# shamanDevel/IsosurfaceSuperresolution

Hardware: AMD Instinct MI355X
Metric: frames/sec (render+4×SR) at 256³→1080p, 1/2/4/8 GPU; PSNR vs ref (higher is better)
Workload: dtype f32 (fp32 tensors and accumulation; each product as three fp16 MFMAs on split operands, error vs fp64 = the fp32 kernels')

## Files before the change

### isosurfacesuperresolution_amd/csrc/sr_conv_ups3.h

```cpp
#pragma once
#include "sr_split_common.h"

#ifndef U3_LFETCH_ROW
#define U3_LFETCH_ROW 2
#endif
#ifndef U3_SPLANE
#define U3_SPLANE 0
#endif
#ifndef U3_WDMA
#define U3_WDMA 1
#endif
#ifndef U3_CARRY
#define U3_CARRY 2
#endif
#ifndef U3_APREF
#define U3_APREF 0
#endif
#ifndef U3_LR_CS
#define U3_LR_CS 114
#endif

namespace {

constexpr int U3_PART = 2 * SP_PIX;
constexpr int U3_PUNITS = 2 * U3_PART;
constexpr int U3_WROW = 3 * 128;
constexpr int U3_WUNITS = (U3_SPLANE ? 3 : 2) * U3_WROW;
constexpr int U3_LDS_BYTES = (U3_PUNITS + (U3_WDMA ? 2 : 1) * U3_WUNITS) * 16;

__global__ __launch_bounds__(S_THREADS, 3) void conv3x3_split_ups3_kernel(const SplitConvParams p)
{
    extern __shared__ u32x4 patch[];
    u32x4* const wbuf = patch + U3_PUNITS;
    const int tid = threadIdx.x, lane = tid & 63, wave = tid >> 6;
    const int j = lane & 31, h = lane >> 5;
    int bid;
    {
        const int nwg = gridDim.x, q = nwg >> 3, r = nwg & 7, xcd = blockIdx.x & 7;
        bid = (xcd < r ? xcd * (q + 1) : r * (q + 1) + (xcd - r) * q) + (blockIdx.x >> 3);
    }
    const int tx = bid % p.tilesX; bid /= p.tilesX;
    const int ty = bid % p.tilesY, n = bid / p.tilesY;
    const int oy0 = ty * ST_H, ox0 = tx * ST_W;
    const rsrc_t xrs = __builtin_amdgcn_make_buffer_rsrc(const_cast<float*>(p.x + (size_t)n * p.xImage), 0,
                                                         (int)((size_t)p.Cin * p.xPlane * 4), 0x00020000);
    const unsigned planeBytes = (unsigned)p.xPlane * 4u;
    unsigned long long st0 = 0, st1 = 0, st2 = 0;
    if (p.stamps) st0 = __builtin_amdgcn_s_memrealtime();

    const rsrc_t wrs = __builtin_amdgcn_make_buffer_rsrc(const_cast<u32x4*>(p.wq + 1), 0, 9 * p.ksteps * 4096, 0x00020000);
    u32x4* const wdst = wbuf + (tid >> 7) * U3_WROW + (tid & 127);
    u32x4 wreg[3];
    const rsrc_t w3rs = __builtin_amdgcn_make_buffer_rsrc(const_cast<u32x4*>(p.wq + 1 + 9 * p.ksteps * 256), 0, 9 * p.ksteps * 2048, 0x00020000);
    u32x4 wreg3[2];
    auto wfetch = [&](int step) {
        if (step >= 3 * p.ksteps) return;
        const int ks = step / 3, dy = step - 3 * ks;
#pragma unroll
        for (int i = 0; i < 3; ++i) wreg[i] = __builtin_amdgcn_raw_buffer_load_b128(wrs, tid * 16, ((3 * dy + i) * p.ksteps + ks) * 4096, 0);
        if (U3_SPLANE) {
#pragma unroll
            for (int k = 0; k < 2; ++k) {
                const int e = tid + 256 * k;
                wreg3[k] = __builtin_amdgcn_raw_buffer_load_b128(w3rs, (int)(e < 384 ? (unsigned)(e & 127) * 16u : BAD_OFFSET), ((3 * dy + (e >> 7)) * p.ksteps + ks) * 2048, 0);
            }
        }
    };
    auto wpark = [&]() {
#pragma unroll
        for (int i = 0; i < 3; ++i) wdst[i * 128] = wreg[i];
        if (U3_SPLANE) {
            wbuf[2 * U3_WROW + tid] = wreg3[0];
            if (tid < 128) wbuf[2 * U3_WROW + 256 + tid] = wreg3[1];
        }
    };

    constexpr int LR_H = ST_H / 2 + 2, LR_W = ST_W / 2 + 2;
    constexpr int LQ = (ST_W / 2 + 8) / 4;
    constexpr int LUNITS = 16 * LR_H * LQ;
    constexpr int LR_CS = U3_LR_CS;
    constexpr int QR = SP_H / 2, QC = SP_W / 2, UQ = QR * QC;
    float* tmp = reinterpret_cast<float*>(wbuf);
    const int wv = __builtin_amdgcn_readfirstlane(wave);
    auto wdma = [&](int step) {
        if (step >= 3 * p.ksteps) return;
        const int ks = step / 3, dy = step - 3 * ks;
#pragma unroll
        for (int k = 0; k < 3; ++k) {
            const int idx = wv + 4 * k, i = idx >> 2, part = (idx >> 1) & 1, half = idx & 1;
            __builtin_amdgcn_raw_ptr_buffer_load_lds(wrs, (isr_lvoid_t*)(wbuf + (step & 1) * U3_WUNITS + part * U3_WROW + i * 128 + half * 64), 16,
                                                     lane * 16, (((3 * dy + i) * p.ksteps + ks) * 256 + part * 128 + half * 64) * 16, 0, 0);
        }
    };
    const int ly0 = oy0 / 2 - 1, lx0 = ox0 / 2 - 1;
    u32x4 v[3];
    auto lfetch = [&](int cin0) {
#pragma unroll
        for (int k = 0; k < 3; ++k) {
            const int u = tid + k * S_THREADS;
            const int c = u / (LR_H * LQ), rem = u - c * (LR_H * LQ);
            const int r = rem / LQ, q = rem - r * LQ;
            const int iy = ly0 + r, ix = ox0 / 2 - 4 + 4 * q;
            const bool ok = u < LUNITS && (unsigned)iy < (unsigned)p.Hin && (unsigned)ix < (unsigned)p.Win;
            v[k] = __builtin_amdgcn_raw_buffer_load_b128(xrs, (int)(ok ? (unsigned)(cin0 + c) * planeBytes + (unsigned)(iy * p.Win + ix) * 4u
                                                                       : BAD_OFFSET), 0, 0);
        }
    };
    auto lpark = [&]() {
#pragma unroll
        for (int k = 0; k < 3; ++k) {
            const int u = tid + k * S_THREADS;
            if (u >= LUNITS) continue;
            const int c = u / (LR_H * LQ), rem = u - c * (LR_H * LQ);
            const int r = rem / LQ, q = rem - r * LQ;
            const float4 f = __builtin_bit_cast(float4, v[k]);
            float* dst = tmp + c * LR_CS + r * LR_W + 4 * q - 3;
            if (q > 0) dst[0] = f.x;
            if (q > 0 && q < LQ - 1) { dst[1] = f.y; dst[2] = f.z; }
            if (q < LQ - 1) dst[3] = f.w;
        }
    };
    const bool interior = oy0 >= 2 && oy0 + ST_H + 2 <= p.H && ox0 >= 2 && ox0 + ST_W + 2 <= p.W;
    auto interpolate = [&]() {
        _Float16* const patch16 = reinterpret_cast<_Float16*>(patch);
        for (int u = tid; u < 4 * UQ; u += S_THREADS) {
            const int g4 = u & 3, q = u >> 2;
            const int kr = q / QC, kc = q - kr * QC;
            f16x4 h00, h01, h10, h11, l00, l01, l10, l11;
            if (interior) {
                const float* ta = tmp + (g4 * 4) * LR_CS + kr * LR_W + kc;
#pragma unroll
                for (int e = 0; e < 4; ++e) {
                    const float a0 = ta[e * LR_CS], a1 = ta[e * LR_CS + 1];
                    const float b0 = ta[e * LR_CS + LR_W], b1 = ta[e * LR_CS + LR_W + 1];
                    const float al = isr_blend(0.75f, a0, 0.25f, a1), ar = isr_blend(0.25f, a0, 0.75f, a1);
                    const float bl = isr_blend(0.75f, b0, 0.25f, b1), br = isr_blend(0.25f, b0, 0.75f, b1);
                    _Float16 vh, vl;
                    split16x(isr_blend(0.75f, al, 0.25f, bl), vh, vl); h00[e] = vh; l00[e] = vl;
                    split16x(isr_blend(0.75f, ar, 0.25f, br), vh, vl); h01[e] = vh; l01[e] = vl;
                    split16x(isr_blend(0.25f, al, 0.75f, bl), vh, vl); h10[e] = vh; l10[e] = vl;
                    split16x(isr_blend(0.25f, ar, 0.75f, br), vh, vl); h11[e] = vh; l11[e] = vl;
                }
            } else {
                const int Yu = oy0 - 1 + 2 * kr, Xl = ox0 - 1 + 2 * kc;
                const bool oku = (unsigned)Yu < (unsigned)p.H, okd = (unsigned)(Yu + 1) < (unsigned)p.H;
                const bool okl = (unsigned)Xl < (unsigned)p.W, okr = (unsigned)(Xl + 1) < (unsigned)p.W;
                int y0, y1, x0, x1, t0, t1; float lyu, lyd, lxl, lxr, t;
                isr_src_index(oku ? Yu : Yu + 1, 0.5f, p.Hin, y0, y1, t);
                isr_src_index(okl ? Xl : Xl + 1, 0.5f, p.Win, x0, x1, t);
                isr_src_index(Yu, 0.5f, p.Hin, t0, t1, lyu);
                isr_src_index(Yu + 1, 0.5f, p.Hin, t0, t1, lyd);
                isr_src_index(Xl, 0.5f, p.Win, t0, t1, lxl);
                isr_src_index(Xl + 1, 0.5f, p.Win, t0, t1, lxr);
                const float hyu = 1.f - lyu, hyd = 1.f - lyd, hxl = 1.f - lxl, hxr = 1.f - lxr;
                y0 = min(max(y0 - ly0, 0), LR_H - 1); y1 = min(max(y1 - ly0, 0), LR_H - 1);
                x0 = min(max(x0 - lx0, 0), LR_W - 1); x1 = min(max(x1 - lx0, 0), LR_W - 1);
                const float* ta = tmp + (g4 * 4) * LR_CS + y0 * LR_W;
                const float* tb = tmp + (g4 * 4) * LR_CS + y1 * LR_W;
#pragma unroll
                for (int e = 0; e < 4; ++e) {
                    const float a0 = ta[e * LR_CS + x0], a1 = ta[e * LR_CS + x1];
                    const float b0 = tb[e * LR_CS + x0], b1 = tb[e * LR_CS + x1];
                    const float al = isr_blend(hxl, a0, lxl, a1), ar = isr_blend(hxr, a0, lxr, a1);
                    const float bl = isr_blend(hxl, b0, lxl, b1), br = isr_blend(hxr, b0, lxr, b1);
                    _Float16 vh, vl;
                    split16x(isr_blend(hyu, al, lyu, bl), vh, vl); h00[e] = vh; l00[e] = vl;
                    split16x(isr_blend(hyu, ar, lyu, br), vh, vl); h01[e] = vh; l01[e] = vl;
                    split16x(isr_blend(hyd, al, lyd, bl), vh, vl); h10[e] = vh; l10[e] = vl;
                    split16x(isr_blend(hyd, ar, lyd, br), vh, vl); h11[e] = vh; l11[e] = vl;
                }
                const f16x4 z = {(_Float16)0.0f, (_Float16)0.0f, (_Float16)0.0f, (_Float16)0.0f};
                if (!(oku && okl)) { h00 = z; l00 = z; }
                if (!(oku && okr)) { h01 = z; l01 = z; }
                if (!(okd && okl)) { h10 = z; l10 = z; }
                if (!(okd && okr)) { h11 = z; l11 = z; }
            }
            _Float16* d = patch16 + ((size_t)((g4 >> 1) * SP_PIX + (2 * kr) * SP_W + 2 * kc)) * 8 + (g4 & 1) * 4;
            *reinterpret_cast<f16x4*>(d) = h00;
            *reinterpret_cast<f16x4*>(d + 8) = h01;
            *reinterpret_cast<f16x4*>(d + SP_W * 8) = h10;
            *reinterpret_cast<f16x4*>(d + SP_W * 8 + 8) = h11;
            *reinterpret_cast<f16x4*>(d + U3_PART * 8) = l00;
            *reinterpret_cast<f16x4*>(d + U3_PART * 8 + 8) = l01;
            *reinterpret_cast<f16x4*>(d + (U3_PART + SP_W) * 8) = l10;
            *reinterpret_cast<f16x4*>(d + (U3_PART + SP_W) * 8 + 8) = l11;
        }
    };

    f32x16 acc[2][2];
#pragma unroll
    for (int cb = 0; cb < 2; ++cb)
#pragma unroll
        for (int r = 0; r < 2; ++r)
#pragma unroll
            for (int i = 0; i < 16; ++i) acc[cb][r][i] = 0.0f;

    lfetch(0);
    if (U3_WDMA) {
        wdma(0);
#pragma unroll 1
        for (int ks = 0; ks < p.ksteps; ++ks) {
            tmp = reinterpret_cast<float*>(wbuf + ((3 * ks + 1) & 1) * U3_WUNITS);
            lpark();
            __syncthreads();
            if (!(p.dbg & 2)) interpolate();
            f16x8 carry[3], carryo[3];
#pragma unroll
            for (int dy = 0; dy < 3; ++dy) {
                asm volatile("s_waitcnt vmcnt(0)" ::: "memory");
                __syncthreads();
                wdma(3 * ks + dy + 1);
                if (dy == U3_LFETCH_ROW && ks + 1 < p.ksteps) lfetch(16 * (ks + 1));
                if (!(p.dbg & 1)) {
                    const u32x4* wl = wbuf + ((3 * ks + dy) & 1) * U3_WUNITS + h * 64 + j;
                    const u32x4* bl = patch + h * SP_PIX + (wave * 2 + dy) * SP_W + j;
                    f16x8 na0h, na0l, na1h, na1l;
                    if (U3_APREF) {
                        na0h = __builtin_bit_cast(f16x8, wl[0]); na0l = __builtin_bit_cast(f16x8, wl[U3_WROW]);
                        na1h = __builtin_bit_cast(f16x8, wl[32]); na1l = __builtin_bit_cast(f16x8, wl[U3_WROW + 32]);
                    }
#pragma unroll
                    for (int dx = 0; dx < 3; ++dx) {
                        f16x8 a0h, a0l, a1h, a1l;
                        if (U3_APREF) {
                            a0h = na0h; a0l = na0l; a1h = na1h; a1l = na1l;
                            if (dx < 2) {
                                na0h = __builtin_bit_cast(f16x8, wl[(dx + 1) * 128]); na0l = __builtin_bit_cast(f16x8, wl[U3_WROW + (dx + 1) * 128]);
                                na1h = __builtin_bit_cast(f16x8, wl[(dx + 1) * 128 + 32]); na1l = __builtin_bit_cast(f16x8, wl[U3_WROW + (dx + 1) * 128 + 32]);
                                __builtin_amdgcn_sched_barrier(0);
                            }
                        } else {
                            a0h = __builtin_bit_cast(f16x8, wl[dx * 128]);
                            a0l = __builtin_bit_cast(f16x8, wl[U3_WROW + dx * 128]);
                            a1h = __builtin_bit_cast(f16x8, wl[dx * 128 + 32]);
                            a1l = __builtin_bit_cast(f16x8, wl[U3_WROW + dx * 128 + 32]);
                        }
                        const f16x8 a0s = a0h * (_Float16)0.00048828125f;
                        const f16x8 a1s = a1h * (_Float16)0.00048828125f;
#pragma unroll
                        for (int r = 0; r < 2; ++r) {
                            const f16x8 bh = (U3_CARRY && r == 0 && dy > 0) ? carry[dx] : __builtin_bit_cast(f16x8, bl[r * SP_W + dx]);
                            const f16x8 bo = (U3_CARRY == 2 && r == 0 && dy > 0) ? carryo[dx] : __builtin_bit_cast(f16x8, bl[U3_PART + r * SP_W + dx]);
                            if (U3_CARRY && r == 1) carry[dx] = bh;
                            if (U3_CARRY == 2 && r == 1) carryo[dx] = bo;
                            acc[0][r] = mfma16(a0l, bh, acc[0][r]);
                            acc[0][r] = mfma16(a0s, bo, acc[0][r]);
                            acc[0][r] = mfma16(a0h, bh, acc[0][r]);
                            acc[1][r] = mfma16(a1l, bh, acc[1][r]);
                            acc[1][r] = mfma16(a1s, bo, acc[1][r]);
                            acc[1][r] = mfma16(a1h, bh, acc[1][r]);
                        }
                    }
                }
            }
            __syncthreads();
        }
    } else {
    wfetch(0);
#pragma unroll 1
    for (int ks = 0; ks < p.ksteps; ++ks) {
        lpark();
        __syncthreads();
        if (!(p.dbg & 2)) interpolate();
        __syncthreads();
        if (p.stamps && ks == 0) st1 = __builtin_amdgcn_s_memrealtime();
#pragma unroll 1
        for (int dy = 0; dy < 3; ++dy) {
            wpark();
            __syncthreads();
            wfetch(3 * ks + dy + 1);
            if (dy == U3_LFETCH_ROW && ks + 1 < p.ksteps) lfetch(16 * (ks + 1));
            if (!(p.dbg & 1)) {
                const u32x4* wl = wbuf + h * 64 + j;
                const u32x4* bl = patch + h * SP_PIX + (wave * 2 + dy) * SP_W + j;
#pragma unroll
                for (int dx = 0; dx < 3; ++dx) {
                    const f16x8 a0h = __builtin_bit_cast(f16x8, wl[dx * 128]);
                    const f16x8 a0l = __builtin_bit_cast(f16x8, wl[U3_WROW + dx * 128]);
                    const f16x8 a1h = __builtin_bit_cast(f16x8, wl[dx * 128 + 32]);
                    const f16x8 a1l = __builtin_bit_cast(f16x8, wl[U3_WROW + dx * 128 + 32]);
                    const f16x8 a0s = U3_SPLANE ? __builtin_bit_cast(f16x8, wl[2 * U3_WROW + dx * 128]) : a0h * (_Float16)0.00048828125f;
                    const f16x8 a1s = U3_SPLANE ? __builtin_bit_cast(f16x8, wl[2 * U3_WROW + dx * 128 + 32]) : a1h * (_Float16)0.00048828125f;
#pragma unroll
                    for (int r = 0; r < 2; ++r) {
                        const f16x8 bh = __builtin_bit_cast(f16x8, bl[r * SP_W + dx]);
                        const f16x8 bo = __builtin_bit_cast(f16x8, bl[U3_PART + r * SP_W + dx]);
                        acc[0][r] = mfma16(a0l, bh, acc[0][r]);
                        acc[0][r] = mfma16(a0s, bo, acc[0][r]);
                        acc[0][r] = mfma16(a0h, bh, acc[0][r]);
                        acc[1][r] = mfma16(a1l, bh, acc[1][r]);
                        acc[1][r] = mfma16(a1s, bo, acc[1][r]);
                        acc[1][r] = mfma16(a1h, bh, acc[1][r]);
                    }
                }
            }
            __syncthreads();
        }
    }
    }

    if (p.stamps) st2 = __builtin_amdgcn_s_memrealtime();
    if (p.dbg & 8) {
        if (acc[0][0][0] == 123.456f) p.ps[0] = u32x4{1u, 2u, 3u, 4u};
    } else if (p.ps) split_epilogue_ps(p, acc, oy0, ox0, 0, true, wave, j, h);
    else split_epilogue<true>(p, acc, patch, n, oy0, ox0, 0, true, lane, wave, j, h);
    if (p.stamps && tid == 0) {
        asm volatile("s_waitcnt vmcnt(0)" ::: "memory");
        const unsigned long long st3 = __builtin_amdgcn_s_memrealtime();
        unsigned long long* o = p.stamps + (size_t)blockIdx.x * 4;
        o[0] = st0; o[1] = st1; o[2] = st2; o[3] = st3;
    }
}

}

static int isr_launch_split_ups3(const SplitConvParams& p, unsigned nwg, hipStream_t s, hipEvent_t e0, hipEvent_t e1)
{
    if (p.Cin <= 0 || (p.Cin & 15) || p.coutPad != 64 || p.Cout != 64 || p.cgroups != 1 || p.xps) return -1;
    if (!p.ps && ((p.W | p.yPlane | p.rPlane) & 3)) return -1;
    static bool attr = false;
    if (!attr) { (void)hipFuncSetAttribute((const void*)conv3x3_split_ups3_kernel, hipFuncAttributeMaxDynamicSharedMemorySize, U3_LDS_BYTES); attr = true; }
    if (e0 || e1) hipExtLaunchKernelGGL(conv3x3_split_ups3_kernel, dim3(nwg), dim3(S_THREADS), U3_LDS_BYTES, s, e0, e1, 0, p);
    else hipLaunchKernelGGL(conv3x3_split_ups3_kernel, dim3(nwg), dim3(S_THREADS), U3_LDS_BYTES, s, p);
    return hipGetLastError() == hipSuccess ? 0 : -2;
}
```

Before: 600.1.

## Stream low-res input tile into LDS via buffer-load-to-LDS DMA

Adds a U3_LDMA path, on by default, that loads the low-resolution input tile directly into a dedicated LDS staging region with buffer_load_lds. This replaces the register fetch followed by an LDS park, and it drops the end-of-iteration barrier in favour of a waitcnt plus barrier at the top of each k-step. The aim is to free VGPRs and remove the park stores, at the cost of extra LDS per workgroup. A host-side occupancy check refuses to launch if fewer than three blocks fit per CU. The loads are scalar 4-byte per-lane DMAs, which may issue many more memory instructions than the previous 16-byte loads.

```diff
diff --git a/isosurfacesuperresolution_amd/csrc/sr_conv_ups3.h b/isosurfacesuperresolution_amd/csrc/sr_conv_ups3.h
--- a/isosurfacesuperresolution_amd/csrc/sr_conv_ups3.h
+++ b/isosurfacesuperresolution_amd/csrc/sr_conv_ups3.h
@@ -9,6 +9,9 @@
 #endif
 #ifndef U3_WDMA
 #define U3_WDMA 1
+#endif
+#ifndef U3_LDMA
+#define U3_LDMA 1
 #endif
 #ifndef U3_CARRY
 #define U3_CARRY 2
@@ -26,7 +29,10 @@
 constexpr int U3_PUNITS = 2 * U3_PART;
 constexpr int U3_WROW = 3 * 128;
 constexpr int U3_WUNITS = (U3_SPLANE ? 3 : 2) * U3_WROW;
-constexpr int U3_LDS_BYTES = (U3_PUNITS + (U3_WDMA ? 2 : 1) * U3_WUNITS) * 16;
+constexpr int U3_TMP_BYTES = 16 * U3_LR_CS * 4;
+constexpr int U3_LDS_BYTES = (U3_PUNITS + (U3_WDMA ? 2 : 1) * U3_WUNITS) * 16 + (U3_LDMA ? U3_TMP_BYTES : 0);
+static_assert(!U3_LDMA || U3_WDMA, "U3_LDMA is a variant of the U3_WDMA loop");
+static_assert(3 * ((U3_LDS_BYTES + 1279) / 1280 * 1280) <= 163840, "conv3x3_split_ups3_kernel no longer fits a CU three times");
 
 __global__ __launch_bounds__(S_THREADS, 3) void conv3x3_split_ups3_kernel(const SplitConvParams p)
 {
@@ -80,7 +86,7 @@
     constexpr int LUNITS = 16 * LR_H * LQ;
     constexpr int LR_CS = U3_LR_CS;
     constexpr int QR = SP_H / 2, QC = SP_W / 2, UQ = QR * QC;
-    float* tmp = reinterpret_cast<float*>(wbuf);
+    float* tmp = reinterpret_cast<float*>(wbuf + (U3_LDMA ? 2 * U3_WUNITS : 0));
     const int wv = __builtin_amdgcn_readfirstlane(wave);
     auto wdma = [&](int step) {
         if (step >= 3 * p.ksteps) return;
@@ -93,6 +99,23 @@
         }
     };
     const int ly0 = oy0 / 2 - 1, lx0 = ox0 / 2 - 1;
+    unsigned lvoff[2];
+#pragma unroll
+    for (int k = 0; k < 2; ++k) {
+        const int e = lane + 64 * k, r = e / LR_W, iy = ly0 + r, ix = lx0 + e - r * LR_W;
+        const bool ok = e < LR_H * LR_W && (unsigned)iy < (unsigned)p.Hin && (unsigned)ix < (unsigned)p.Win;
+        lvoff[k] = ok ? (unsigned)(iy * p.Win + ix) * 4u : BAD_OFFSET;
+    }
+    auto ldma = [&](int cin0) {
+#pragma unroll
+        for (int c = 0; c < 4; ++c)
+            __builtin_amdgcn_raw_ptr_buffer_load_lds(xrs, (isr_lvoid_t*)(tmp + (4 * wv + c) * LR_CS), 4, (int)lvoff[0], (int)((unsigned)(cin0 + 4 * wv + c) * planeBytes), 0, 0);
+        if (lane < LR_H * LR_W - 64) {
+#pragma unroll
+            for (int c = 0; c < 4; ++c)
+                __builtin_amdgcn_raw_ptr_buffer_load_lds(xrs, (isr_lvoid_t*)(tmp + (4 * wv + c) * LR_CS + 64), 4, (int)lvoff[1], (int)((unsigned)(cin0 + 4 * wv + c) * planeBytes), 0, 0);
+        }
+    };
     u32x4 v[3];
     auto lfetch = [&](int cin0) {
 #pragma unroll
@@ -195,14 +218,19 @@
 #pragma unroll
             for (int i = 0; i < 16; ++i) acc[cb][r][i] = 0.0f;
 
-    lfetch(0);
+    if (U3_LDMA) ldma(0); else lfetch(0);
     if (U3_WDMA) {
         wdma(0);
 #pragma unroll 1
         for (int ks = 0; ks < p.ksteps; ++ks) {
-            tmp = reinterpret_cast<float*>(wbuf + ((3 * ks + 1) & 1) * U3_WUNITS);
-            lpark();
-            __syncthreads();
+            if (U3_LDMA) {
+                asm volatile("s_waitcnt vmcnt(0)" ::: "memory");
+                __syncthreads();
+            } else {
+                tmp = reinterpret_cast<float*>(wbuf + ((3 * ks + 1) & 1) * U3_WUNITS);
+                lpark();
+                __syncthreads();
+            }
             if (!(p.dbg & 2)) interpolate();
             f16x8 carry[3], carryo[3];
 #pragma unroll
@@ -210,7 +238,7 @@
                 asm volatile("s_waitcnt vmcnt(0)" ::: "memory");
                 __syncthreads();
                 wdma(3 * ks + dy + 1);
-                if (dy == U3_LFETCH_ROW && ks + 1 < p.ksteps) lfetch(16 * (ks + 1));
+                if (dy == U3_LFETCH_ROW && ks + 1 < p.ksteps) { if (U3_LDMA) ldma(16 * (ks + 1)); else lfetch(16 * (ks + 1)); }
                 if (!(p.dbg & 1)) {
                     const u32x4* wl = wbuf + ((3 * ks + dy) & 1) * U3_WUNITS + h * 64 + j;
                     const u32x4* bl = patch + h * SP_PIX + (wave * 2 + dy) * SP_W + j;
@@ -253,8 +281,9 @@
                     }
                 }
             }
-            __syncthreads();
-        }
+            if (!U3_LDMA) __syncthreads();
+        }
+        if (U3_LDMA) __syncthreads();
     } else {
     wfetch(0);
 #pragma unroll 1
@@ -319,7 +348,12 @@
     if (p.Cin <= 0 || (p.Cin & 15) || p.coutPad != 64 || p.Cout != 64 || p.cgroups != 1 || p.xps) return -1;
     if (!p.ps && ((p.W | p.yPlane | p.rPlane) & 3)) return -1;
     static bool attr = false;
-    if (!attr) { (void)hipFuncSetAttribute((const void*)conv3x3_split_ups3_kernel, hipFuncAttributeMaxDynamicSharedMemorySize, U3_LDS_BYTES); attr = true; }
+    if (!attr) {
+        (void)hipFuncSetAttribute((const void*)conv3x3_split_ups3_kernel, hipFuncAttributeMaxDynamicSharedMemorySize, U3_LDS_BYTES);
+        int perCU = 0;
+        if (hipOccupancyMaxActiveBlocksPerMultiprocessor(&perCU, (const void*)conv3x3_split_ups3_kernel, S_THREADS, U3_LDS_BYTES) != hipSuccess || perCU < 3) return -2;
+        attr = true;
+    }
     if (e0 || e1) hipExtLaunchKernelGGL(conv3x3_split_ups3_kernel, dim3(nwg), dim3(S_THREADS), U3_LDS_BYTES, s, e0, e1, 0, p);
     else hipLaunchKernelGGL(conv3x3_split_ups3_kernel, dim3(nwg), dim3(S_THREADS), U3_LDS_BYTES, s, p);
     return hipGetLastError() == hipSuccess ? 0 : -2;
```

Result: no change. 602.0 (median of 6 runs) (+0.3%).
